# facebook/transform360

Hardware: NVIDIA H100
Metric: Mpixels/s 8K equirect->cubemap bicubic (input-plane pixels consumed per second) (higher is better)
Workload: dtype u8

## Files before the change

### include/transform360_b200.h

```cpp
#ifndef TRANSFORM360_B200_EXT_H
#define TRANSFORM360_B200_EXT_H

#include "Transform360/VideoFrameTransformHandler.h"

#ifdef __cplusplus
extern "C" {
#endif

typedef struct T360HostPlan T360HostPlan;

T360HostPlan* T360B200_hostPlanCreate(const FrameTransformContext* ctx, int inputWidth, int inputHeight,
                                      int outputWidth, int outputHeight);
void T360B200_hostPlanDestroy(T360HostPlan* plan);
int T360B200_hostPlanInfo(const T360HostPlan* plan, int info[6]);
const float* T360B200_hostPlanMap(const T360HostPlan* plan);
const int32_t* T360B200_hostPlanSamples(const T360HostPlan* plan);
int T360B200_hostPlanGather(T360HostPlan* plan, int info[10], const int32_t** jobs, const int32_t** records,
                            const uint32_t** compact);
int T360B200_hostPlanPoleCaps(T360HostPlan* plan, int info[4], const int32_t** capJobs, const uint32_t** capRecords,
                              const int32_t** launchJobs);
int T360B200_dealLanes(int interpolationAlg, int n, const int32_t* phases, int32_t* laneOf, int32_t* copyOf);
int T360B200_weightImage(int interpolationAlg, const uint8_t** image);
int T360B200_hostPlanBlurLists(T360HostPlan* const* plans, int numPlans, int width, int height, int layout[15],
                               const uint8_t** image);
int T360B200_hostPlanSegment(const T360HostPlan* plan, int i, int rect[4], int numTaps[2], const float** kx,
                             const float** ky);
int T360B200_remapTable(int interpolationAlg, const int16_t** table);

int T360B200_transformFramePlaneAsync(VideoFrameTransform* transform, const uint8_t* deviceInput,
                                      uint8_t* deviceOutput, int inputWidth, int inputHeight, int inputPitch,
                                      int outputWidth, int outputHeight, int outputPitch,
                                      int transformMatPlaneIndex, void* cudaStream);
int T360B200_transformFrameAsync(VideoFrameTransform* transform, int numPlanes, const uint8_t* const* deviceInputs,
                                 uint8_t* const* deviceOutputs, const int* inputWidths, const int* inputHeights,
                                 const int* inputPitches, const int* outputWidths, const int* outputHeights,
                                 const int* outputPitches, void* cudaStream);
int T360B200_lowPassPlaneAsync(VideoFrameTransform* transform, const uint8_t* deviceInput, uint8_t* deviceOutput,
                               int width, int height, int inputPitch, int outputPitch,
                               int transformMatPlaneIndex, void* cudaStream);
int T360B200_reconfigure(VideoFrameTransform* transform, const FrameTransformContext* ctx);
typedef struct T360View {
  float yaw, pitch, hfov, vfov;
} T360View;
// ... 33 lines not shown
```

### transform360_b200/build.py

```python
from __future__ import annotations

import os
import shutil
import subprocess
import sys
from pathlib import Path

PKG = Path(__file__).resolve().parent
ROOT = PKG.parent
CSRC = PKG / "csrc"
LIB_DIR = PKG / "lib"
LIB = LIB_DIR / "libTransform360.so"
SOURCES = ["geometry.cpp", "lowpass_plan.cpp", "lowpass_jobs.cpp", "sampling.cpp", "gather_plan.cpp", "kernels.cu", "gather_frame.cu", "view_gather.cu", "video_frame_transform.cpp"]
ARCH = ["-gencode", "arch=compute_90a,code=sm_90a"]


def nvcc_path() -> str:
    p = shutil.which("nvcc") or "/usr/local/cuda/bin/nvcc"
    if not Path(p).exists():
        raise FileNotFoundError("nvcc not found (needed to build libTransform360.so)")
    return p


def needs_build() -> bool:
    if not LIB.exists():
        return True
    t = LIB.stat().st_mtime
    deps = list(CSRC.glob("*")) + list((ROOT / "include").rglob("*.h")) + [Path(__file__)]
    return any(d.stat().st_mtime > t for d in deps)


def build(force: bool = False, verbose: bool = False, defines: tuple = (), out: Path | None = None) -> Path:
    out = out or LIB
    if not force and not defines and not needs_build():
        return LIB
    LIB_DIR.mkdir(exist_ok=True)
# ... 65 lines not shown
```

### transform360_b200/csrc/gather_frame.cu

```cuda
#include "gather_common.cuh"

#include <cuda.h>

#include <algorithm>
#include <cstring>
#include <utility>

namespace t360 {

namespace {

template <class F, int... I>
__device__ __forceinline__ void staticForImpl(F&& f, std::integer_sequence<int, I...>) {
  (f(std::integral_constant<int, I>{}), ...);
}
template <int N, class F>
__device__ __forceinline__ void staticFor(F&& f) {
  staticForImpl(f, std::make_integer_sequence<int, N>{});
}

template <int IMM>
__device__ __forceinline__ uint32_t ldsWordImm(uint32_t addr) {
  uint32_t v;
  asm volatile("ld.shared.u32 %0, [%1+%2];" : "=r"(v) : "r"(addr), "n"(IMM));
// ... 102 lines not shown
  staticFor<8>([&](auto V) {
    constexpr int v = decltype(V)::value;
    const uint4 wt = ldsVecImm<0>(wAddr + (first ^ (uint32_t)(v * kDiagonalStep)));
    const uint32_t b0 = p2 ? B[v ^ 4].b[0] : B[v].b[0], b1 = p2 ? B[v ^ 4].b[1] : B[v].b[1];
    acc = dp2aLo(wt.x, b0, acc); acc = dp2aHi(wt.y, b0, acc);
    acc = dp2aLo(wt.z, b1, acc); acc = dp2aHi(wt.w, b1, acc);
  });
  return acc;
}
template <int K, int VS>
__device__ __forceinline__ int foldPixel(const RowBytes<K> (&W)[K], uint32_t wAddr, uint32_t field) {
  if constexpr (K == 8) return foldRowsRotated<VS>(W, wAddr, field);
  else return foldRows<K, VS>(W, wAddr + slotOffset<K>(field));
}
__device__ __forceinline__ int biasedToByte(int acc) { return min(max(acc >> 15, 0), 255); }


__device__ __forceinline__ uint32_t packBytes(int hi, int lo) {
  uint32_t r;
  asm("cvt.pack.sat.u8.s32.b32 %0, %1, %2, %3;" : "=r"(r) : "r"(hi), "r"(lo), "r"(0));
  return r;
}

template <int K, int PITCH, int VS, int ROWS, bool ZERO>
__device__ __forceinline__ void computeShareJob(uint8_t* dst, int dstPitch, uint32_t stageAddr, const uint4 (&rec)[ROWS / 8],
                                                uint32_t header, uint32_t wAddr) {
  static_assert(PITCH % 4 == 0 && (K == 4 || K == 8) && ROWS % 8 == 0, "");
  uint32_t base = stageAddr + (header & 0x7ffcu);
  const int sh = (int)(header << 3);
  RowBytes<K> W[K];
  staticFor<K>([&](auto R) { W[decltype(R)::value] = loadRow<K, decltype(R)::value * PITCH>(base, sh); });
  int accPrev = 0;
  staticFor<ROWS>([&](auto J) {
    constexpr int j = decltype(J)::value;
    const uint4& block = rec[j >> 3];
    const uint32_t word = ((j >> 1) & 3) == 0 ? block.x : (((j >> 1) & 3) == 1 ? block.y : (((j >> 1) & 3) == 2 ? block.z : block.w));
    const uint32_t r = (j & 1) ? word >> 16 : word;
    if constexpr (j > 0 && !ZERO) {
      const bool two = (r & 1u) != 0;
      const RowBytes<K> below = loadRow<K, (j - 1 + K) * PITCH>(base, sh);
      RowBytes<K> below2 = below;
      if (two) below2 = loadRow<K, (j + K) * PITCH>(base, sh);
#pragma unroll
      for (int q = 0; q + 2 < K; ++q)
#pragma unroll
        for (int i = 0; i < (K == 8 ? 2 : 1); ++i) W[q].b[i] = two ? W[q + 2].b[i] : W[q + 1].b[i];
#pragma unroll
      for (int i = 0; i < (K == 8 ? 2 : 1); ++i) W[K - 2].b[i] = two ? below.b[i] : W[K - 1].b[i];
      W[K - 1] = below2;
      if (two) base += PITCH;
    }
    if constexpr (j > 0 && ZERO) {
      const uint32_t d = r & 3u;
      RowBytes<K> below = W[K - 1], below2 = W[K - 1];
      if (d != 0) below = loadRow<K, K * PITCH>(base, sh);
      if (d == 2) below2 = loadRow<K, (K + 1) * PITCH>(base, sh);
#pragma unroll
      for (int q = 0; q + 2 < K; ++q)
#pragma unroll
        for (int i = 0; i < (K == 8 ? 2 : 1); ++i) W[q].b[i] = d == 0 ? W[q].b[i] : (d == 1 ? W[q + 1].b[i] : W[q + 2].b[i]);
#pragma unroll
      for (int i = 0; i < (K == 8 ? 2 : 1); ++i) {
        W[K - 2].b[i] = d == 0 ? W[K - 2].b[i] : (d == 1 ? W[K - 1].b[i] : below.b[i]);
        W[K - 1].b[i] = d == 0 ? W[K - 1].b[i] : (d == 1 ? below.b[i] : below2.b[i]);
      }
      base += d * PITCH;
    }
    const int acc = foldPixel<K, VS>(W, wAddr, r & kSlotFieldMask) >> 15;
    if constexpr (j & 1) {
      const uint32_t pair = packBytes(acc, accPrev);
      dst[(size_t)(j - 1) * dstPitch] = (uint8_t)pair;
      dst[(size_t)j * dstPitch] = (uint8_t)(pair >> 8);
    } else {
      accPrev = acc;
    }
  });
}

template <int K, int PITCH, int VS>
__device__ __forceinline__ void computeTileJob(const PlaneView& pv, uint32_t stageAddr, int outX, int outY, const uint4& rec,
                                               uint32_t wAddr, int warp) {
  static_assert(PITCH % 4 == 0, "");
  const int y0 = outY + warp * kTilePatchH;
  const int dstPitch = pv.dstPitch, dstW = pv.dstW, dstH = pv.dstH;
  uint8_t* const dstRow = pv.dst + (size_t)y0 * dstPitch + outX;
  const uint32_t words[4] = {rec.x, rec.y, rec.z, rec.w};
  staticFor<kRowsPerPatchStep>([&](auto J) {
    constexpr int j = decltype(J)::value;
    const uint32_t w = words[j];
    const int col = kTilePatchW * j + ((int)(w >> 16) & (kTilePatchW - 1)), row = (int)(w >> 19) & (kTilePatchH - 1);
    if (!(w & kRecordSkip) && outX + col < dstW && y0 + row < dstH) {
// ... 138 lines not shown
      }
      int4 h;
      h.x = __shfl_sync(0xffffffffu, batch.x, pos); h.y = __shfl_sync(0xffffffffu, batch.y, pos);
      h.z = __shfl_sync(0xffffffffu, batch.z, pos); h.w = __shfl_sync(0xffffffffu, batch.w, pos);
      ++pos;
      const int kind = (h.y >> kJobKindShift) & kJobKindMask;
      mbarWait(empty + st, phase ^ 1);
      const bool twoStages = kind == kJobClass1 || kind == kJobSeam;
      if (twoStages) {
        if (st == S - 1) {
          if (lane == 0) postEmptyJob(kJobNop);
          advance();
          mbarWait(empty + st, phase ^ 1);
        }
        mbarWait(empty + st + 1, phase ^ 1);
      }
      if (lane == 0) {
        unsigned char* rec = groupBase + S * kStage + st * kRec;
        *reinterpret_cast<int4*>(rec) = h;
        if (kind == kJobExit) {
          mbarArrive(full + st);
        } else {
          const int pl = h.y >> kJobPlaneShift;
          const uint32_t recBytes = (uint32_t)jobRecordBytes(K, kind, h.x);
          if (kind == kJobBorder) {
            mbarExpectTx(full + st, recBytes);
          } else {
            const int cls = boxClassOf(kind), variant = jobBoxVariant(h.z), boxX = jobBoxX(h.z), boxY = jobBoxY(h.z);
            const uint32_t boxBytes = (uint32_t)(stageBoxW(K, cls) * boxVariantRows(K, cls, variant));
            mbarExpectTx(full + st, (kind == kJobSeam ? 2 : 1) * boxBytes + recBytes);
            tmaLoadBox(groupBase + st * kStage, &maps.map[pl][cls][variant], boxX, boxY, full + st);
            if (kind == kJobSeam)
              tmaLoadBox(groupBase + (st + 1) * kStage, &maps.map[pl][0][variant], boxX - planes[pl].srcW, boxY, full + st);
          }
          bulkCopyToShared(rec + 128, planes[pl].records + (unsigned)h.w, recBytes, full + st);
        }
      }
      advance();
      if (twoStages) {
        if (lane == 0) postEmptyJob(kJobNop);
        advance();
      }
      __syncwarp();
      if (kind == kJobExit) break;
    }
    if (lane == 0 && atomicAdd(jobs.claimCounter + 1, 1) == (int)(gridDim.x * GROUPS) - 1) {
      jobs.claimCounter[0] = 0;
// ... 3 lines not shown
    return;
  }

  const int group = warpId / kGroupWarps, warp = warpId % kGroupWarps;
  unsigned char* groupBase = smem + L::kWeights + group * L::kGroupBytes;
  const uint32_t boxAddr = smemAddr(groupBase), recAddr = smemAddr(groupBase + S * kStage);
  uint64_t* full = barBase + group * 2 * S;
  uint64_t* empty = full + S;
  const uint32_t wAddr = smemAddr(wsmem);
  mbarWait(weightBar, 0);
  asm volatile("griddepcontrol.wait;" ::: "memory");
  auto now = []() { unsigned long long t; asm volatile("mov.u64 %0, %globaltimer;" : "=l"(t)); return t; };
  unsigned long long* trace = jobs.trace && warp == 0 && lane == 0 ? jobs.trace + (size_t)(blockIdx.x * GROUPS + group) * kTraceJobsPerGroup * 4 : nullptr;
  uint32_t traced = 0;
  for (uint32_t st = 0, phase = 0;;) {
    unsigned long long* const row = trace && traced < kTraceJobsPerGroup ? trace + traced * 4 : nullptr;
    if (row) row[0] = now();
    mbarWait(full + st, phase);
    if (row) row[1] = now();
    const uint32_t rec = recAddr + st * kRec;
    const uint4 h = ldsVec(rec);
    const int kind = ((int)h.y >> kJobKindShift) & kJobKindMask;
    if (kind == kJobExit) break;
    const int outX = (int)h.x & ~kJobQuadMask, outY = (int)h.y & kJobRowMask;
    const PlaneView& pv = planes[(int)h.y >> kJobPlaneShift];
    if (kind == kJobShare || kind == kJobShareStay) {
      if constexpr (K >= 4) {
        const uint32_t mine = rec + 128 + warp * shareWarpRecordBytes(K);
        uint4 r[shareRows(K) / 8];
#pragma unroll
        for (int b = 0; b < shareRows(K) / 8; ++b) r[b] = ldsVec(mine + b * 512 + lane * 16);
        const uint32_t header = ldsWord(mine + shareRows(K) / 8 * 512 + lane * 4);
        uint8_t* dst = pv.dst + (size_t)(outY + (warp >> 1) * shareRows(K)) * pv.dstPitch + (outX + (warp & 1) * 32 + (int)(header >> kRecordColumnShift));
        if (kind == kJobShare) computeShareJob<K, stageBoxW(K, 2), VS, shareRows(K), false>(dst, pv.dstPitch, boxAddr + st * kStage, r, header, wAddr);
        else computeShareJob<K, stageBoxW(K, 2), VS, shareRows(K), true>(dst, pv.dstPitch, boxAddr + st * kStage, r, header, wAddr);
      }
    } else if (kind == kJobClass0) {
      uint4 r;
      const int quad = ((int)h.x & kJobQuadMask) - 1;
      if (quad < 0) {
        r = ldsVec(rec + 128 + warp * 512 + lane * 16);
      } else {
        r = make_uint4(kRecordSkip, kRecordSkip, kRecordSkip, kRecordSkip);
        if ((warp >> 2) == (quad >> 1)) {
          const uint2 v = ldsVec2Imm<0>(rec + 128 + (warp & 3) * 256 + lane * 8);
          if (quad & 1) { r.z = v.x; r.w = v.y; } else { r.x = v.x; r.y = v.y; }
        }
      }
      computeTileJob<K, stageBoxW(K, 0), VS>(pv, boxAddr + st * kStage, outX, outY, r, wAddr, warp);
    } else if (kind == kJobClass1) {
      computeTileJob<K, stageBoxW(K, 1), VS>(pv, boxAddr + st * kStage, outX, outY, ldsVec(rec + 128 + warp * 512 + lane * 16), wAddr, warp);
    } else if (kind == kJobSeam) {
      {
        uint4* a = reinterpret_cast<uint4*>(groupBase + st * kStage);
        const uint4* b = reinterpret_cast<const uint4*>(groupBase + (st + 1) * kStage);
        for (int i = warp * 32 + lane; i < (int)(kBox0 / 16); i += kGroupThreads) {
          uint4 x = a[i];
          const uint4 y = b[i];
// ... 83 lines not shown
```

### transform360_b200/csrc/kernels.cuh

```cuda
#pragma once

#include <cuda_runtime.h>

#include <cstdint>

#include "flat_view.h"
#include "oriented_view.h"

namespace t360 {

struct GatherParams {
  const uint8_t* src;
  int srcW, srcH, srcPitch;
  uint8_t* dst;
  int dstW, dstH, dstPitch;
  const int2* samples;
  int tilesPerRow;
  const int16_t* weights;
  int kernelSize;
  int transparent;
};

struct GatherJob {
  int outX, outY;
// ... 63 lines not shown
}
__host__ __device__ constexpr int weightBankGroups(int k) { return k == 2 ? 16 : 8; }
__host__ __device__ constexpr int weightLanesPerPass(int k) { return k == 2 ? 16 : 8; }

__host__ __device__ constexpr int shareWarpRecordBytes(int k) { return shareRows(k) / 8 * 32 * 16 + 32 * 4; }
__host__ __device__ constexpr int shareJobRecordBytes(int k) { return kGroupWarps * shareWarpRecordBytes(k); }
constexpr int kTileJobRecordBytes = kGroupWarps * 32 * 16;
constexpr int kQuadJobRecordBytes = kGroupWarps / 2 * 32 * 8;
__host__ __device__ constexpr int tileJobRecordBytes(int outXField) { return (outXField & kJobQuadMask) ? kQuadJobRecordBytes : kTileJobRecordBytes; }
__host__ __device__ constexpr int stageRecordBytes(int k) {
  return 128 + (shareJobRecordBytes(k) > kTileJobRecordBytes ? shareJobRecordBytes(k) : kTileJobRecordBytes);
}
constexpr int kCapStepBytes = 32 * 8, kBorderPixelBytes = 16;
__host__ __device__ constexpr int capJobMaxSteps(int k) { return (stageRecordBytes(k) - 128) / kCapStepBytes; }
__host__ __device__ constexpr int borderJobMaxPixels(int k) { return (stageRecordBytes(k) - 128) / kBorderPixelBytes; }
__host__ __device__ constexpr int jobRecordBytes(int k, int kind, int outXField) {
  return kind == kJobShare || kind == kJobShareStay ? shareJobRecordBytes(k)
         : kind == kJobCap                          ? outXField * kCapStepBytes
         : kind == kJobBorder                       ? outXField * kBorderPixelBytes
                                                    : tileJobRecordBytes(outXField);
}
constexpr int kRecordColumnShift = 27;

constexpr int kMaxFramePlanes = 3;
struct PlaneView {
  const uint8_t* src;
  uint8_t* dst;
  const uint4* records;
  int srcW, srcH, srcPitch;
  int dstW, dstH, dstPitch;
};
struct FrameGatherParams {
  PlaneView plane[kMaxFramePlanes];
  const uint4* weightImage;
  int kernelSize, numPlanes;
};

__host__ __device__ constexpr int gatherThreads(int k) { return k == 8 ? 512 : 256; }
__host__ __device__ constexpr int gatherTileH(int k) { return gatherThreads(k) / 32 * 4; }

struct StagedParams {
  const GatherJob* tiles;
  int numTiles;
  int* claimCounter;
  unsigned long long* trace;
};
// ... 120 lines not shown
```

### transform360_b200/csrc/video_frame_transform.cpp

```cpp
#include <cuda.h>
#include <cuda_runtime.h>

#include <algorithm>
#include <climits>
#include <cmath>
#include <cstdio>
#include <cstdlib>
#include <cstring>
#include <map>
#include <memory>
#include <mutex>
#include <new>
#include <shared_mutex>
#include <stdexcept>
#include <string>
#include <thread>
#include <vector>

#include "host_plan.h"
#include "gather_plan.h"
#include "kernels.cuh"
#include "lowpass_jobs.h"
#include "transform360_b200.h"

#define T360_API extern "C" __attribute__((visibility("default")))

namespace {

using t360::BlurJob;
using t360::GatherJob;
using t360::HostPlan;
using t360::StripJob;

struct CudaFail {
  cudaError_t err;
  const char* what;
};

#define CU(call)                                       \
  do {                                                 \
    cudaError_t e__ = (call);                          \
    if (e__ != cudaSuccess) throw CudaFail{e__, #call}; \
// ... 1066 lines not shown
      const std::vector<uint8_t> image = t360::buildWeightImage(k, host);
      weightImages_[k].reserve(image.size());
      CU(cudaMemcpy(weightImages_[k].ptr, image.data(), image.size(), cudaMemcpyHostToDevice));
    }
    return buf.ptr;
  }

  DevicePlan upload(HostIndexPlan& p, const FrameTransformContext& ctx) {
    const HostPlan& h = p.host;
    DevicePlan d;
    d.inW = h.inW; d.inH = h.inH; d.outW = h.outW; d.outH = h.outH; d.mapW = h.mapW; d.mapH = h.mapH;
    d.kernelSize = h.kernelSize;
    d.transparent = h.transparentBorder;
    d.stereoFormat = ctx.input_stereo_format;
    if (d.kernelSize > 0) {
      deviceWeights(ctx.interpolation_alg);
      t360::GatherPlan& g = p.gather;
      d.tilesPerRow = g.tilesPerRow;
      d.samples.reserve(g.records.size());
      CU(cudaMemcpy(d.samples.ptr, g.records.data(), g.records.size() * sizeof(int2), cudaMemcpyHostToDevice));
      d.numStaged = g.totalStaged();
      d.numBorder = g.numBorder;
      d.numJobs = static_cast<int>(g.launchJobs.size());
      if (!g.launchJobs.empty()) {
        d.gatherJobs.reserve(g.launchJobs.size());
        CU(cudaMemcpy(d.gatherJobs.ptr, g.launchJobs.data(), g.launchJobs.size() * sizeof(GatherJob), cudaMemcpyHostToDevice));
      }
      if (!g.compact.empty() || !g.capRecords.empty()) {
        d.records.reserve(g.compact.size() + g.capRecords.size());
        if (!g.compact.empty())
          CU(cudaMemcpy(d.records.ptr, g.compact.data(), g.compact.size() * sizeof(uint32_t), cudaMemcpyHostToDevice));
        if (!g.capRecords.empty())
          CU(cudaMemcpy(d.records.ptr + g.compact.size(), g.capRecords.data(), g.capRecords.size() * sizeof(uint32_t), cudaMemcpyHostToDevice));
      }
      d.hostJobs = std::move(g.launchJobs);
      d.jobNeedRows = std::move(g.launchNeedRows);
      d.jobRects = std::move(g.launchRects);
    }
    d.lowPass = ctx.enable_low_pass_filter != 0;
    if (d.lowPass) {
      d.segments = h.segments;
      d.planTaps = h.taps;
      buildBlurSet(d.segments, d.planTaps, h.inW, h.inH, d.stereoFormat, d.blur);
    }
    d.resizeNeeded = h.resize.needed;
    if (d.resizeNeeded) resizeFor(d, d.outW, d.outH);
    if (d.kernelSize > 0 && t360::orientedLayouts(ctx)) {
      const std::vector<float> t = t360::buildSphereTables(t360::sphereGeometry(ctx, h.mapW, h.mapH, h.inW, h.inH, h.kernelSize));
      if (!t.empty()) {
        d.sphereTables.reserve(t.size());
        CU(cudaMemcpy(d.sphereTables.ptr, t.data(), t.size() * sizeof(float), cudaMemcpyHostToDevice));
      }
    }
    return d;
  }

  const DevicePlan::Resize& resizeFor(const DevicePlan& plan, int outW, int outH) {
    std::lock_guard<std::mutex> lock(lazyMu_);
// ... 431 lines not shown

T360_API int VideoFrameTransform_generateMapForPlane(VideoFrameTransform* transform, int inputWidth, int inputHeight,
                                                     int outputWidth, int outputHeight, int transformMatPlaneIndex) {
  if (!transform) return 0;
  return transform->generateMapForPlane(inputWidth, inputHeight, outputWidth, outputHeight, transformMatPlaneIndex);
}

T360_API int VideoFrameTransform_transformFramePlane(VideoFrameTransform* transform, uint8_t* inputData,
                                                     uint8_t* outputData, int inputWidth, int inputHeight,
                                                     int inputWidthWithPadding, int outputWidth, int outputHeight,
                                                     int outputWidthWithPadding, int transformMatPlaneIndex,
                                                     int imagePlaneIndex) {
  if (!transform) return 0;
  return transform->transformFramePlane(inputData, outputData, inputWidth, inputHeight, inputWidthWithPadding,
                                        outputWidth, outputHeight, outputWidthWithPadding, transformMatPlaneIndex,
                                        imagePlaneIndex);
}

struct T360HostPlan {
  HostPlan plan;
  t360::GatherPlan gather;
  bool gatherBuilt = false;
  std::vector<uint8_t> blurImage;
};

T360_API T360HostPlan* T360B200_hostPlanCreate(const FrameTransformContext* ctx, int inW, int inH, int outW, int outH) {
  if (!ctx) return nullptr;
  std::unique_ptr<T360HostPlan> p(new (std::nothrow) T360HostPlan);
  if (!p) return nullptr;
  try {
    if (!t360::buildHostPlan(*ctx, inW, inH, outW, outH, p->plan)) return nullptr;
  } catch (const std::exception& ex) {
    std::printf("Could not build the host plan. Error: %s\n", ex.what());
    return nullptr;
  }
  return p.release();
}
T360_API void T360B200_hostPlanDestroy(T360HostPlan* plan) { delete plan; }
T360_API int T360B200_hostPlanInfo(const T360HostPlan* plan, int info[6]) {
  if (!plan || !info) return 0;
  info[0] = plan->plan.mapW; info[1] = plan->plan.mapH;
  info[2] = static_cast<int>(plan->plan.segments.size());
  info[3] = static_cast<int>(plan->plan.taps.size());
  info[4] = plan->plan.kernelSize;
  info[5] = 0;
  return 1;
// ... 13 lines not shown
  } catch (const std::exception& ex) {
    std::printf("Could not build the gather plan. Error: %s\n", ex.what());
    return 0;
  }
  const t360::GatherPlan& g = plan->gather;
  info[0] = g.tilesPerRow; info[1] = g.tileRows; info[2] = g.tileH; info[3] = static_cast<int>(g.jobs.size());
  info[4] = g.numStaged[0]; info[5] = g.numStaged[1]; info[6] = g.numSeam; info[7] = g.numGeneral;
  info[8] = g.numShare; info[9] = static_cast<int>(g.compact.size());
  if (jobs) *jobs = g.jobs.empty() ? nullptr : reinterpret_cast<const int32_t*>(g.jobs.data());
  if (records) *records = reinterpret_cast<const int32_t*>(g.records.data());
  if (compact) *compact = g.compact.empty() ? nullptr : g.compact.data();
  return 1;
}
T360_API int T360B200_hostPlanPoleCaps(T360HostPlan* plan, int info[4], const int32_t** capJobs, const uint32_t** capRecords,
                                       const int32_t** launchJobs) {
  int gatherInfo[10];
  if (!plan || !info || !T360B200_hostPlanGather(plan, gatherInfo, nullptr, nullptr, nullptr)) return 0;
  const t360::GatherPlan& g = plan->gather;
  info[0] = g.numCap; info[1] = g.numBorder; info[2] = static_cast<int>(g.capRecords.size());
  info[3] = static_cast<int>(g.launchJobs.size());
  if (capJobs) *capJobs = g.capJobs.empty() ? nullptr : reinterpret_cast<const int32_t*>(g.capJobs.data());
  if (capRecords) *capRecords = g.capRecords.empty() ? nullptr : g.capRecords.data();
  if (launchJobs) *launchJobs = g.launchJobs.empty() ? nullptr : reinterpret_cast<const int32_t*>(g.launchJobs.data());
  return 1;
}
T360_API int T360B200_hostPlanBlurLists(T360HostPlan* const* plans, int numPlans, int width, int height, int layout[15],
                                        const uint8_t** image) {
  if (!plans || numPlans < 1 || numPlans > t360::kMaxFramePlanes || !layout || !image) return 0;
  for (int p = 0; p < numPlans; ++p)
    if (!plans[p]) return 0;
  try {
    t360::BlurLists lists[t360::kMaxFramePlanes];
    const t360::BlurLists* planes[t360::kMaxFramePlanes];
    bool clear = false;
    for (int p = 0; p < numPlans; ++p) {
      const HostPlan& h = plans[p]->plan;
      bool c = false;
      t360::buildBlurLists(h.segments, h.taps, width > 0 ? width : h.inW, height > 0 ? height : h.inH, h.ctx.input_stereo_format, lists[p], &c);
      clear = clear || c;
      planes[p] = &lists[p];
    }
    std::vector<uint8_t>& img = plans[0]->blurImage;
    img.clear();
    const t360::BlurLayout l = t360::packBlurLists(numPlans > 1 ? t360::mergeBlurLists(planes, numPlans) : lists[0], img, img);
    const long long v[15] = {l.numStrips[0], l.numStrips[1], l.numStrips[2], l.numTiles, l.numDirect, l.numTaps, l.tileSmem, clear,
                             static_cast<long long>(l.stripAt[0]), static_cast<long long>(l.stripAt[1]), static_cast<long long>(l.stripAt[2]),
// ... 164 lines not shown
```

### transform360_b200/handler.py

```python
from __future__ import annotations

import ctypes as C
import os
from pathlib import Path

import numpy as np

PKG = Path(__file__).resolve().parent
LIB_PATH = PKG / "lib" / "libTransform360.so"

LAYOUT_CUBEMAP_32, LAYOUT_CUBEMAP_23_OFFCENTER, LAYOUT_FLAT_FIXED, LAYOUT_EQUIRECT = 0, 1, 2, 3
LAYOUT_BARREL, LAYOUT_BARREL_SPLIT, LAYOUT_EAC_32, LAYOUT_N = 4, 5, 6, 7
STEREO_FORMAT_TB, STEREO_FORMAT_LR, STEREO_FORMAT_MONO, STEREO_FORMAT_GUESS, STEREO_FORMAT_N = 0, 1, 2, 3, 4
NEAREST, LINEAR, CUBIC, LANCZOS4 = 0, 1, 2, 4


class FrameTransformContext(C.Structure):
    _fields_ = [
        ("input_layout", C.c_int), ("output_layout", C.c_int),
        ("input_stereo_format", C.c_int), ("output_stereo_format", C.c_int),
        ("vflip", C.c_int), ("input_expand_coef", C.c_float), ("expand_coef", C.c_float),
        ("interpolation_alg", C.c_int), ("width_scale_factor", C.c_float),
        ("height_scale_factor", C.c_float), ("fixed_yaw", C.c_float), ("fixed_pitch", C.c_float),
        ("fixed_roll", C.c_float), ("fixed_hfov", C.c_float), ("fixed_vfov", C.c_float),
# ... 63 lines not shown
    L.VideoFrameTransform_delete.argtypes = [vp]
    L.VideoFrameTransform_generateMapForPlane.restype = ci
    L.VideoFrameTransform_generateMapForPlane.argtypes = [vp] + [ci] * 5
    L.VideoFrameTransform_transformFramePlane.restype = ci
    L.VideoFrameTransform_transformFramePlane.argtypes = [vp, vp, vp] + [ci] * 8
    L.T360B200_hostPlanCreate.restype = vp
    L.T360B200_hostPlanCreate.argtypes = [C.POINTER(FrameTransformContext)] + [ci] * 4
    L.T360B200_hostPlanDestroy.restype = None
    L.T360B200_hostPlanDestroy.argtypes = [vp]
    L.T360B200_hostPlanInfo.restype = ci
    L.T360B200_hostPlanInfo.argtypes = [vp, C.POINTER(ci)]
    L.T360B200_hostPlanMap.restype = vp
    L.T360B200_hostPlanMap.argtypes = [vp]
    L.T360B200_hostPlanSamples.restype = vp
    L.T360B200_hostPlanSamples.argtypes = [vp]
    L.T360B200_hostPlanSegment.restype = ci
    L.T360B200_hostPlanSegment.argtypes = [vp, ci, C.POINTER(ci), C.POINTER(ci), C.POINTER(vp), C.POINTER(vp)]
    L.T360B200_hostPlanGather.restype = ci
    L.T360B200_hostPlanGather.argtypes = [vp, C.POINTER(ci), C.POINTER(vp), C.POINTER(vp), C.POINTER(vp)]
    L.T360B200_hostPlanPoleCaps.restype = ci
    L.T360B200_hostPlanBlurLists.restype = ci
    L.T360B200_hostPlanBlurLists.argtypes = [vp, ci, ci, ci, C.POINTER(ci), C.POINTER(vp)]
    L.T360B200_hostPlanPoleCaps.argtypes = [vp, C.POINTER(ci), C.POINTER(vp), C.POINTER(vp), C.POINTER(vp)]
    L.T360B200_weightImage.restype = ci
    L.T360B200_weightImage.argtypes = [ci, C.POINTER(vp)]
    L.T360B200_remapTable.restype = ci
    L.T360B200_remapTable.argtypes = [ci, C.POINTER(vp)]
    L.T360B200_transformFramePlaneAsync.restype = ci
    L.T360B200_transformFramePlaneAsync.argtypes = [vp, vp, vp] + [ci] * 7 + [vp]
    L.T360B200_transformFrameAsync.restype = ci
    L.T360B200_transformFrameAsync.argtypes = [vp, ci, vp, vp] + [vp] * 6 + [vp]
    L.T360B200_lowPassPlaneAsync.restype = ci
    L.T360B200_lowPassPlaneAsync.argtypes = [vp, vp, vp] + [ci] * 5 + [vp]
    L.T360B200_reconfigure.restype = ci
    L.T360B200_reconfigure.argtypes = [vp, C.POINTER(FrameTransformContext)]
    L.T360B200_transformFrameViewAsync.restype = ci
    L.T360B200_transformFrameViewAsync.argtypes = [vp, C.POINTER(T360View), ci, vp, vp] + [vp] * 6 + [vp]
    L.T360B200_viewSamples.restype = ci
    L.T360B200_viewSamples.argtypes = [C.POINTER(FrameTransformContext), C.POINTER(T360View)] + [ci] * 4 + [vp]
    L.T360B200_transformFrameOrientedAsync.restype = ci
    L.T360B200_transformFrameOrientedAsync.argtypes = [vp, C.POINTER(T360Orientation), ci, vp, vp] + [vp] * 6 + [vp]
    L.T360B200_orientedSamples.restype = ci
    L.T360B200_orientedSamples.argtypes = [C.POINTER(FrameTransformContext), C.POINTER(T360Orientation)] + [ci] * 4 + [vp]
    L.T360B200_setPinHostPlanes.restype = None
    L.T360B200_setPinHostPlanes.argtypes = [vp, ci]
    L.T360B200_debugTrace.restype = None
    L.T360B200_debugTrace.argtypes = [vp, ci]
    L.T360B200_debugTraceRead.restype = C.c_ulonglong
    L.T360B200_debugTraceRead.argtypes = [vp, vp, C.c_ulonglong]
    L.T360B200_synchronize.restype = ci
    L.T360B200_synchronize.argtypes = [vp]
    L.T360B200_stream.restype = vp
    L.T360B200_stream.argtypes = [vp]
    L.T360B200_kernelLaunchCount.restype = C.c_ulonglong
    L.T360B200_planDeviceBytes.restype = C.c_ulonglong
    L.T360B200_planDeviceBytes.argtypes = [vp, ci]
    L.T360B200_planTileCounts.restype = ci
    L.T360B200_planTileCounts.argtypes = [vp, ci, C.POINTER(ci)]
    L.T360B200_deviceCount.restype = ci
    L.T360B200_version.restype = C.c_char_p
    if path is None:
        _lib = L
    return L


EXPORTED_SYMBOLS = [
    "VideoFrameTransform_new", "VideoFrameTransform_delete", "VideoFrameTransform_generateMapForPlane",
    "VideoFrameTransform_transformFramePlane", "T360B200_hostPlanCreate", "T360B200_hostPlanDestroy",
    "T360B200_hostPlanInfo", "T360B200_hostPlanMap", "T360B200_hostPlanSamples", "T360B200_hostPlanSegment",
    "T360B200_hostPlanGather", "T360B200_hostPlanPoleCaps", "T360B200_hostPlanBlurLists", "T360B200_weightImage", "T360B200_dealLanes",
    "T360B200_remapTable", "T360B200_transformFramePlaneAsync", "T360B200_transformFrameAsync",
    "T360B200_lowPassPlaneAsync", "T360B200_reconfigure", "T360B200_transformFrameViewAsync", "T360B200_viewSamples",
    "T360B200_transformFrameOrientedAsync", "T360B200_orientedSamples",
    "T360B200_setPinHostPlanes", "T360B200_debugTrace", "T360B200_debugTraceRead", "T360B200_synchronize", "T360B200_stream", "T360B200_kernelLaunchCount", "T360B200_planDeviceBytes",
    "T360B200_planTileCounts", "T360B200_deviceCount", "T360B200_version",
]


class VideoFrameTransform:

    def __init__(self, ctx: FrameTransformContext):
        self._lib = load()
        self.ctx = ctx
        self._h = self._lib.VideoFrameTransform_new(C.byref(ctx))
        if not self._h:
            raise MemoryError("VideoFrameTransform_new returned NULL")

    def close(self):
        if getattr(self, "_h", None):
            self._lib.VideoFrameTransform_delete(self._h)
            self._h = None

    __del__ = close
# ... 150 lines not shown
        if not self._lib.T360B200_hostPlanGather(self._h, info, C.byref(jobs), C.byref(recs), C.byref(comp)):
            raise ValueError("T360B200_hostPlanGather failed")
        tpr, trows, th, nj = info[0], info[1], info[2], info[3]
        n = tpr * trows * th * 32 * 2
        records = np.frombuffer((C.c_int32 * n).from_address(recs.value), np.int32).reshape(tpr * trows, th, 32, 2).copy()
        j = compact = None
        if nj and jobs.value:
            j = np.frombuffer((C.c_int32 * (nj * 4)).from_address(jobs.value), np.int32).reshape(nj, 4).copy()
        if info[9] and comp.value:
            compact = np.frombuffer((C.c_uint32 * info[9]).from_address(comp.value), np.uint32).copy()
        return dict(tiles_per_row=tpr, tile_rows=trows, tile_h=th, jobs=j, records=records, compact=compact,
                    counts=dict(class0=info[4], class1=info[5], seam=info[6], general=info[7], share=info[8]))

    def pole_caps(self):
        info = (C.c_int * 4)()
        jobs, recs, launch = C.c_void_p(), C.c_void_p(), C.c_void_p()
        if not self._lib.T360B200_hostPlanPoleCaps(self._h, info, C.byref(jobs), C.byref(recs), C.byref(launch)):
            raise ValueError("T360B200_hostPlanPoleCaps failed")
        n, m = info[0] + info[1], info[3]
        as_jobs = lambda p, k: np.frombuffer((C.c_int32 * (k * 4)).from_address(p.value), np.int32).reshape(k, 4).copy() if k and p.value else np.zeros((0, 4), np.int32)
        records = np.frombuffer((C.c_uint32 * info[2]).from_address(recs.value), np.uint32).copy() if info[2] and recs.value else np.zeros(0, np.uint32)
        return dict(counts=dict(cap=info[0], border=info[1]), jobs=as_jobs(jobs, n), records=records, launch=as_jobs(launch, m))

    def blur_lists(self, *others, width=0, height=0):
        plans = (C.c_void_p * (1 + len(others)))(self._h, *[o._h for o in others])
        lay, img = (C.c_int * 15)(), C.c_void_p()
        if not self._lib.T360B200_hostPlanBlurLists(plans, len(plans), width, height, lay, C.byref(img)):
            raise ValueError("T360B200_hostPlanBlurLists failed (message on stdout)")
        image = C.string_at(img.value, lay[14]) if lay[14] else b""
        arr = lambda at, n, cols, dt: np.frombuffer(image, dt, n * cols, at).reshape(n, cols).copy()
        return dict(image=image, strips=[arr(lay[8 + c], lay[c], 9, np.int32) for c in range(3)], tiles=arr(lay[11], lay[3], 8, np.int32),
                    direct=arr(lay[12], lay[4], 8, np.int32), taps=np.frombuffer(image, np.float32, lay[5], lay[13]).copy(),
                    offsets=list(lay[8:14]), tile_smem=lay[6], needs_clear=bool(lay[7]))

    def segments(self):
        out = []
        rect, nk = (C.c_int * 4)(), (C.c_int * 2)()
        kx, ky = C.c_void_p(), C.c_void_p()
        for i in range(self.num_segments):
            assert self._lib.T360B200_hostPlanSegment(self._h, i, rect, nk, C.byref(kx), C.byref(ky))
            a = np.frombuffer((C.c_float * nk[0]).from_address(kx.value), np.float32).copy()
            b = np.frombuffer((C.c_float * nk[1]).from_address(ky.value), np.float32).copy()
            out.append((rect[0], rect[1], rect[2], rect[3], a, b))
        return out


# ... 56 lines not shown
```

Measured before the change: 730,900.

## Pack bicubic share-job records into compact per-lane bytes for device streaming

Adds a host-side pass that re-encodes share-job records for the bicubic (K=4) path. For each warp whose rows share one column phase, the per-row 16-bit slot fields become 8-bit step/fracY bytes, with the column phase folded into the header. The kernel decodes these packed records and keeps the old layout only for 'wide' warps, which are flagged by a bitmask in the job's outX. This cuts the record bytes fetched per job into shared memory, at the cost of extra decode ALU work and a 16-bit limit on output columns. It also adds a traffic-measurement script.

```diff
diff --git a/include/transform360_b200.h b/include/transform360_b200.h
--- a/include/transform360_b200.h
+++ b/include/transform360_b200.h
@@ -19,6 +19,7 @@
                             const uint32_t** compact);
 int T360B200_hostPlanPoleCaps(T360HostPlan* plan, int info[4], const int32_t** capJobs, const uint32_t** capRecords,
                               const int32_t** launchJobs);
+int T360B200_hostPlanDeviceRecords(T360HostPlan* plan, int info[2], const int32_t** launchJobs, const uint32_t** words);
 int T360B200_dealLanes(int interpolationAlg, int n, const int32_t* phases, int32_t* laneOf, int32_t* copyOf);
 int T360B200_weightImage(int interpolationAlg, const uint8_t** image);
 int T360B200_hostPlanBlurLists(T360HostPlan* const* plans, int numPlans, int width, int height, int layout[15],
diff --git a/profiles/record_traffic.py b/profiles/record_traffic.py
--- /dev/null
+++ b/profiles/record_traffic.py
@@ -0,0 +1,83 @@
+from __future__ import annotations
+
+import argparse
+import json
+import statistics
+import subprocess
+import sys
+from pathlib import Path
+
+ROOT = Path(__file__).resolve().parents[1]
+sys.path.insert(0, str(ROOT))
+
+
+def gpu_info():
+    q = subprocess.run(["nvidia-smi", "-i", "0", "--query-gpu=name,power.limit,clocks.max.sm", "--format=csv,noheader,nounits"],
+                       capture_output=True, text=True).stdout.strip().split(", ")
+    return {"gpu": q[0], "power_limit_w": float(q[1]), "sm_max_mhz": float(q[2])} if len(q) == 3 else {"gpu": None, "power_limit_w": None}
+
+
+def main():
+    ap = argparse.ArgumentParser()
+    ap.add_argument("--config", default="cfg2", choices=["cfg2", "cfg3", "cfg4"])
+    ap.add_argument("--frames", type=int, default=500, help="frames per timed window")
+    ap.add_argument("--rounds", type=int, default=5, help="alternated windows of each condition")
+    ap.add_argument("--label", default="", help="free text stored with the line (e.g. which build)")
+    ap.add_argument("--out", help="append the JSON line to this file")
+    args = ap.parse_args()
+    import torch
+    import transform360_b200 as t360
+    from bench import CONFIGS
+    from transform360_b200 import synth
+    from transform360_b200.stream import FrameTransformer, StreamSpec
+
+    if not torch.cuda.is_available():
+        sys.exit("needs a CUDA device")
+    info = gpu_info()
+    cfg = CONFIGS[args.config]
+    spec = StreamSpec(cfg["inp"][0], cfg["inp"][1], cfg["out"][0], cfg["out"][1])
+    ft = FrameTransformer(t360.make_context(**dict(cfg["ov"], enable_low_pass_filter=0)), spec)
+    pitch = lambda w: (w + 255) // 256 * 256
+    ring = max(4, -(-200_000_000 // spec.input_pixels_per_frame()))
+    d_in = [[synth.noise_plane_torch(*spec.plane_dims(p)[:2], plane=p, frame=f, device="cuda", pitch=pitch(spec.plane_dims(p)[0]))
+             for p in range(3)] for f in range(ring)]
+    d_out = [[torch.zeros((spec.plane_dims(p)[3], pitch(spec.plane_dims(p)[2])), dtype=torch.uint8, device="cuda") for p in range(3)]
+             for _ in range(2)]
+    args_of = lambda planes: [(t.data_ptr(), t.stride(0)) for t in planes]
+    calls = [[ft.frame_call(args_of(d_in[i]), args_of(d_out[o])) for o in range(2)] for i in range(ring)]
+    st = torch.cuda.Stream()
+
+    def window(repeat):
+        for i in range(10):
+            assert calls[0 if repeat else i % ring][i % 2](st.cuda_stream)
+        a, b = torch.cuda.Event(enable_timing=True), torch.cuda.Event(enable_timing=True)
+        a.record(st)
+        for i in range(args.frames):
+            assert calls[0 if repeat else i % ring][i % 2](st.cuda_stream)
+        b.record(st)
+        b.synchronize()
+        return a.elapsed_time(b) / args.frames
+
+    torch.cuda.synchronize()
+    times = {"ring": [], "repeat": []}
+    for _ in range(args.rounds):
+        times["ring"].append(window(False))
+        times["repeat"].append(window(True))
+    summary = {k: {"ms": [round(x, 5) for x in v], "median_ms": round(statistics.median(v), 5), "min_ms": round(min(v), 5),
+                   "max_ms": round(max(v), 5)} for k, v in times.items()}
+    separated = summary["repeat"]["max_ms"] < summary["ring"]["min_ms"]
+    line = dict(info, label=args.label, config=args.config, frames=args.frames, rounds=args.rounds, ring_frames=ring,
+                input_bytes_per_frame=spec.input_pixels_per_frame(), output_bytes_per_frame=spec.output_pixels_per_frame(),
+                plan_device_bytes=[ft.vft.plan_device_bytes(i) for i in (0, 1)], conditions=summary,
+                repeat_faster_outside_spread=separated,
+                repeat_saving=round(1 - summary["repeat"]["median_ms"] / summary["ring"]["median_ms"], 4))
+    ft.close()
+    out = json.dumps(line)
+    print(out)
+    if args.out:
+        with open(args.out, "a") as f:
+            f.write(out + "\n")
+
+
+if __name__ == "__main__":
+    main()
diff --git a/transform360_b200/build.py b/transform360_b200/build.py
--- a/transform360_b200/build.py
+++ b/transform360_b200/build.py
@@ -11,7 +11,7 @@
 CSRC = PKG / "csrc"
 LIB_DIR = PKG / "lib"
 LIB = LIB_DIR / "libTransform360.so"
-SOURCES = ["geometry.cpp", "lowpass_plan.cpp", "lowpass_jobs.cpp", "sampling.cpp", "gather_plan.cpp", "kernels.cu", "gather_frame.cu", "view_gather.cu", "video_frame_transform.cpp"]
+SOURCES = ["geometry.cpp", "lowpass_plan.cpp", "lowpass_jobs.cpp", "sampling.cpp", "gather_plan.cpp", "device_records.cpp", "kernels.cu", "gather_frame.cu", "view_gather.cu", "video_frame_transform.cpp"]
 ARCH = ["-gencode", "arch=compute_90a,code=sm_90a"]
 
 
diff --git a/transform360_b200/csrc/device_records.cpp b/transform360_b200/csrc/device_records.cpp
--- /dev/null
+++ b/transform360_b200/csrc/device_records.cpp
@@ -0,0 +1,71 @@
+#include "device_records.h"
+
+#include <climits>
+#include <stdexcept>
+
+namespace t360 {
+namespace {
+
+constexpr uint32_t kFracYBits = 0x3e00;
+
+uint32_t shareRecord(const uint32_t* warp, int lane, int j) { return (warp[lane * 4 + (j >> 1)] >> (16 * (j & 1))) & 0xffffu; }
+
+uint32_t columnPhase(int k, uint32_t columnField) {
+  const int copy = static_cast<int>(columnField >> 14) & 1, inCopy = static_cast<int>(columnField >> 4) & 31;
+  const int slot = copy ? ((inCopy & ~7) | ((inCopy - copy) & 7)) : inCopy;
+  const int fracX = ((slot & 15) << 1) | ((slot >> 4) & 1);
+  if (static_cast<uint32_t>(weightSlotField(k, fracX, copy)) != columnField) throw std::logic_error("device records: not a slot field");
+  return static_cast<uint32_t>(fracX | (copy << 5));
+}
+
+unsigned packShareJob(int k, const uint32_t* job, std::vector<uint32_t>& out) {
+  unsigned wide = 0;
+  for (int w = 0; w < kGroupWarps; ++w) {
+    const uint32_t* warp = job + static_cast<size_t>(w) * (shareWarpRecordBytes(k) / 4);
+    for (int lane = 0; lane < 32 && !(wide >> w & 1u); ++lane)
+      for (int j = 1; j < shareRows(k); ++j)
+        if ((shareRecord(warp, lane, j) ^ shareRecord(warp, lane, 0)) & kSlotFieldMask & ~kFracYBits) wide |= 1u << w;
+    if (wide >> w & 1u) {
+      out.insert(out.end(), warp, warp + shareWarpRecordBytes(k) / 4);
+      continue;
+    }
+    const uint32_t* headers = warp + shareRows(k) / 8 * 32 * 4;
+    for (int lane = 0; lane < 32; ++lane) {
+      uint32_t bytes[2] = {0, 0};
+      for (int j = 0; j < shareRows(k); ++j) {
+        const uint32_t r = shareRecord(warp, lane, j);
+        if (r & ~(kSlotFieldMask | 3u)) throw std::logic_error("device records: share step out of range");
+        bytes[j >> 2] |= (((r & kFracYBits) >> 9) << 3 | (r & 3u)) << (8 * (j & 3));
+      }
+      out.push_back(bytes[0]);
+      out.push_back(bytes[1]);
+    }
+    for (int lane = 0; lane < 32; ++lane) {
+      const uint32_t phase = columnPhase(k, shareRecord(warp, lane, 0) & kSlotFieldMask & ~kFracYBits);
+      out.push_back(headers[lane] | (phase & 31u) << kShareFracXShift | (phase >> 5) << kShareCopyShift);
+    }
+  }
+  return wide;
+}
+
+}
+
+void buildDeviceRecords(const GatherPlan& g, int k, DeviceRecords& out) {
+  out = DeviceRecords{};
+  out.launchJobs = g.launchJobs;
+  for (GatherJob& job : out.launchJobs) {
+    const int kind = (job.outY >> kJobKindShift) & kJobKindMask;
+    const size_t at = static_cast<size_t>(job.recordOffset) * 4;
+    const uint32_t* src = at < g.compact.size() ? &g.compact[at] : &g.capRecords[at - g.compact.size()];
+    job.recordOffset = static_cast<int>(out.words.size() / 4);
+    if (sharePacked(k) && (kind == kJobShare || kind == kJobShareStay)) {
+      if (job.outX >> kJobShareWideShift) throw std::invalid_argument("device records: share jobs hold 16-bit output columns");
+      job.outX |= static_cast<int>(packShareJob(k, src, out.words)) << kJobShareWideShift;
+    } else {
+      out.words.insert(out.words.end(), src, src + jobRecordBytes(k, kind, job.outX) / 4);
+    }
+    if (out.words.size() / 4 > static_cast<size_t>(INT32_MAX)) throw std::invalid_argument("device records: offsets overflow");
+  }
+}
+
+}
diff --git a/transform360_b200/csrc/device_records.h b/transform360_b200/csrc/device_records.h
--- /dev/null
+++ b/transform360_b200/csrc/device_records.h
@@ -0,0 +1,17 @@
+#pragma once
+
+#include <cstdint>
+#include <vector>
+
+#include "gather_plan.h"
+
+namespace t360 {
+
+struct DeviceRecords {
+  std::vector<GatherJob> launchJobs;
+  std::vector<uint32_t> words;
+};
+
+void buildDeviceRecords(const GatherPlan& g, int k, DeviceRecords& out);
+
+}
diff --git a/transform360_b200/csrc/gather_frame.cu b/transform360_b200/csrc/gather_frame.cu
--- a/transform360_b200/csrc/gather_frame.cu
+++ b/transform360_b200/csrc/gather_frame.cu
@@ -148,10 +148,36 @@
   return r;
 }
 
-template <int K, int PITCH, int VS, int ROWS, bool ZERO>
-__device__ __forceinline__ void computeShareJob(uint8_t* dst, int dstPitch, uint32_t stageAddr, const uint4 (&rec)[ROWS / 8],
+struct CompactShareRecords {
+  uint4 r;
+  template <int j>
+  __device__ __forceinline__ uint32_t rec() const {
+    const uint32_t word = (j >> 1) == 0 ? r.x : ((j >> 1) == 1 ? r.y : ((j >> 1) == 2 ? r.z : r.w));
+    return (j & 1) ? word >> 16 : word;
+  }
+  template <int j>
+  __device__ __forceinline__ uint32_t field() const { return rec<j>() & kSlotFieldMask; }
+  template <int j>
+  __device__ __forceinline__ uint32_t step() const { return rec<j>(); }
+};
+struct PackedShareRecords {
+  uint2 b;
+  uint32_t columnField;
+  template <int j>
+  __device__ __forceinline__ uint32_t field() const {
+    constexpr int s = 8 * (j & 3) + 3 - 9;
+    const uint32_t word = j < 4 ? b.x : b.y;
+    return ((s >= 0 ? word >> s : word << -s) & 0x3e00u) | columnField;
+  }
+  template <int j>
+  __device__ __forceinline__ uint32_t step() const { return (j < 4 ? b.x : b.y) >> (8 * (j & 3)); }
+};
+
+template <int K, int PITCH, int VS, bool ZERO, class Records>
+__device__ __forceinline__ void computeShareJob(uint8_t* dst, int dstPitch, uint32_t stageAddr, const Records& rec,
                                                 uint32_t header, uint32_t wAddr) {
-  static_assert(PITCH % 4 == 0 && (K == 4 || K == 8) && ROWS % 8 == 0, "");
+  constexpr int ROWS = 8;
+  static_assert(PITCH % 4 == 0 && (K == 4 || K == 8) && shareRows(K) == ROWS, "");
   uint32_t base = stageAddr + (header & 0x7ffcu);
   const int sh = (int)(header << 3);
   RowBytes<K> W[K];
@@ -159,9 +185,7 @@
   int accPrev = 0;
   staticFor<ROWS>([&](auto J) {
     constexpr int j = decltype(J)::value;
-    const uint4& block = rec[j >> 3];
-    const uint32_t word = ((j >> 1) & 3) == 0 ? block.x : (((j >> 1) & 3) == 1 ? block.y : (((j >> 1) & 3) == 2 ? block.z : block.w));
-    const uint32_t r = (j & 1) ? word >> 16 : word;
+    const uint32_t r = rec.template step<j>();
     if constexpr (j > 0 && !ZERO) {
       const bool two = (r & 1u) != 0;
       const RowBytes<K> below = loadRow<K, (j - 1 + K) * PITCH>(base, sh);
@@ -192,7 +216,7 @@
       }
       base += d * PITCH;
     }
-    const int acc = foldPixel<K, VS>(W, wAddr, r & kSlotFieldMask) >> 15;
+    const int acc = foldPixel<K, VS>(W, wAddr, rec.template field<j>()) >> 15;
     if constexpr (j & 1) {
       const uint32_t pair = packBytes(acc, accPrev);
       dst[(size_t)(j - 1) * dstPitch] = (uint8_t)pair;
@@ -377,7 +401,7 @@
           mbarArrive(full + st);
         } else {
           const int pl = h.y >> kJobPlaneShift;
-          const uint32_t recBytes = (uint32_t)jobRecordBytes(K, kind, h.x);
+          const uint32_t recBytes = (uint32_t)deviceJobRecordBytes(K, kind, h.x);
           if (kind == kJobBorder) {
             mbarExpectTx(full + st, recBytes);
           } else {
@@ -427,18 +451,31 @@
     const uint4 h = ldsVec(rec);
     const int kind = ((int)h.y >> kJobKindShift) & kJobKindMask;
     if (kind == kJobExit) break;
-    const int outX = (int)h.x & ~kJobQuadMask, outY = (int)h.y & kJobRowMask;
+    const int outX = (int)h.x & kJobOutXMask, outY = (int)h.y & kJobRowMask;
     const PlaneView& pv = planes[(int)h.y >> kJobPlaneShift];
     if (kind == kJobShare || kind == kJobShareStay) {
       if constexpr (K >= 4) {
-        const uint32_t mine = rec + 128 + warp * shareWarpRecordBytes(K);
-        uint4 r[shareRows(K) / 8];
-#pragma unroll
-        for (int b = 0; b < shareRows(K) / 8; ++b) r[b] = ldsVec(mine + b * 512 + lane * 16);
-        const uint32_t header = ldsWord(mine + shareRows(K) / 8 * 512 + lane * 4);
-        uint8_t* dst = pv.dst + (size_t)(outY + (warp >> 1) * shareRows(K)) * pv.dstPitch + (outX + (warp & 1) * 32 + (int)(header >> kRecordColumnShift));
-        if (kind == kJobShare) computeShareJob<K, stageBoxW(K, 2), VS, shareRows(K), false>(dst, pv.dstPitch, boxAddr + st * kStage, r, header, wAddr);
-        else computeShareJob<K, stageBoxW(K, 2), VS, shareRows(K), true>(dst, pv.dstPitch, boxAddr + st * kStage, r, header, wAddr);
+        constexpr int PITCH = stageBoxW(K, 2);
+        const uint32_t wide = h.x >> kJobShareWideShift;
+        const uint32_t mine = sharePacked(K) ? rec + 128 + warp * kPackedShareWarpBytes + __popc(wide & ((1u << warp) - 1u)) * shareWideExtraBytes(K)
+                                             : rec + 128 + warp * shareWarpRecordBytes(K);
+        const uint32_t stageAddr = boxAddr + st * kStage;
+        if (sharePacked(K) && !((wide >> warp) & 1u)) {
+          PackedShareRecords r;
+          r.b = ldsVec2Imm<0>(mine + lane * 8);
+          const uint32_t header = ldsWord(mine + 256 + lane * 4);
+          r.columnField = (uint32_t)weightSlotField(K, (header >> kShareFracXShift) & 31u, (header >> kShareCopyShift) & 1u);
+          uint8_t* dst = pv.dst + (size_t)(outY + (warp >> 1) * shareRows(K)) * pv.dstPitch + (outX + (warp & 1) * 32 + (int)(header >> kRecordColumnShift));
+          if (kind == kJobShare) computeShareJob<K, PITCH, VS, false>(dst, pv.dstPitch, stageAddr, r, header, wAddr);
+          else computeShareJob<K, PITCH, VS, true>(dst, pv.dstPitch, stageAddr, r, header, wAddr);
+        } else {
+          CompactShareRecords r;
+          r.r = ldsVec(mine + lane * 16);
+          const uint32_t header = ldsWord(mine + 512 + lane * 4);
+          uint8_t* dst = pv.dst + (size_t)(outY + (warp >> 1) * shareRows(K)) * pv.dstPitch + (outX + (warp & 1) * 32 + (int)(header >> kRecordColumnShift));
+          if (kind == kJobShare) computeShareJob<K, PITCH, VS, false>(dst, pv.dstPitch, stageAddr, r, header, wAddr);
+          else computeShareJob<K, PITCH, VS, true>(dst, pv.dstPitch, stageAddr, r, header, wAddr);
+        }
       }
     } else if (kind == kJobClass0) {
       uint4 r;
diff --git a/transform360_b200/csrc/kernels.cuh b/transform360_b200/csrc/kernels.cuh
--- a/transform360_b200/csrc/kernels.cuh
+++ b/transform360_b200/csrc/kernels.cuh
@@ -109,6 +109,22 @@
 }
 constexpr int kRecordColumnShift = 27;
 
+__host__ __device__ constexpr bool sharePacked(int k) { return k == 4; }
+constexpr int kShareFracXShift = 16, kShareCopyShift = 21, kJobShareWideShift = 16;
+constexpr int kJobOutXMask = 0xffff & ~kJobQuadMask;
+constexpr int kPackedShareWarpBytes = 32 * 8 + 32 * 4;
+static_assert(shareRows(4) == 8 && shareRows(8) == 8, "packed share records hold 8 rows per warp");
+__host__ __device__ constexpr int shareWideExtraBytes(int k) { return shareWarpRecordBytes(k) - kPackedShareWarpBytes; }
+__host__ __device__ constexpr int packedShareJobRecordBytes(int k, unsigned wideMask) {
+  int n = 0;
+  for (; wideMask; wideMask &= wideMask - 1) ++n;
+  return kGroupWarps * kPackedShareWarpBytes + n * shareWideExtraBytes(k);
+}
+__host__ __device__ constexpr int deviceJobRecordBytes(int k, int kind, int outXField) {
+  return sharePacked(k) && (kind == kJobShare || kind == kJobShareStay) ? packedShareJobRecordBytes(k, (unsigned)outXField >> kJobShareWideShift)
+                                                                        : jobRecordBytes(k, kind, outXField);
+}
+
 constexpr int kMaxFramePlanes = 3;
 struct PlaneView {
   const uint8_t* src;
diff --git a/transform360_b200/csrc/video_frame_transform.cpp b/transform360_b200/csrc/video_frame_transform.cpp
--- a/transform360_b200/csrc/video_frame_transform.cpp
+++ b/transform360_b200/csrc/video_frame_transform.cpp
@@ -18,6 +18,7 @@
 #include <vector>
 
 #include "host_plan.h"
+#include "device_records.h"
 #include "gather_plan.h"
 #include "kernels.cuh"
 #include "lowpass_jobs.h"
@@ -1130,18 +1131,17 @@
       d.numStaged = g.totalStaged();
       d.numBorder = g.numBorder;
       d.numJobs = static_cast<int>(g.launchJobs.size());
-      if (!g.launchJobs.empty()) {
-        d.gatherJobs.reserve(g.launchJobs.size());
-        CU(cudaMemcpy(d.gatherJobs.ptr, g.launchJobs.data(), g.launchJobs.size() * sizeof(GatherJob), cudaMemcpyHostToDevice));
-      }
-      if (!g.compact.empty() || !g.capRecords.empty()) {
-        d.records.reserve(g.compact.size() + g.capRecords.size());
-        if (!g.compact.empty())
-          CU(cudaMemcpy(d.records.ptr, g.compact.data(), g.compact.size() * sizeof(uint32_t), cudaMemcpyHostToDevice));
-        if (!g.capRecords.empty())
-          CU(cudaMemcpy(d.records.ptr + g.compact.size(), g.capRecords.data(), g.capRecords.size() * sizeof(uint32_t), cudaMemcpyHostToDevice));
-      }
-      d.hostJobs = std::move(g.launchJobs);
+      t360::DeviceRecords dr;
+      t360::buildDeviceRecords(g, d.kernelSize, dr);
+      if (!dr.launchJobs.empty()) {
+        d.gatherJobs.reserve(dr.launchJobs.size());
+        CU(cudaMemcpy(d.gatherJobs.ptr, dr.launchJobs.data(), dr.launchJobs.size() * sizeof(GatherJob), cudaMemcpyHostToDevice));
+      }
+      if (!dr.words.empty()) {
+        d.records.reserve(dr.words.size());
+        CU(cudaMemcpy(d.records.ptr, dr.words.data(), dr.words.size() * sizeof(uint32_t), cudaMemcpyHostToDevice));
+      }
+      d.hostJobs = std::move(dr.launchJobs);
       d.jobNeedRows = std::move(g.launchNeedRows);
       d.jobRects = std::move(g.launchRects);
     }
@@ -1619,6 +1619,8 @@
   t360::GatherPlan gather;
   bool gatherBuilt = false;
   std::vector<uint8_t> blurImage;
+  t360::DeviceRecords deviceRecords;
+  bool deviceRecordsBuilt = false;
 };
 
 T360_API T360HostPlan* T360B200_hostPlanCreate(const FrameTransformContext* ctx, int inW, int inH, int outW, int outH) {
@@ -1678,6 +1680,25 @@
   if (capJobs) *capJobs = g.capJobs.empty() ? nullptr : reinterpret_cast<const int32_t*>(g.capJobs.data());
   if (capRecords) *capRecords = g.capRecords.empty() ? nullptr : g.capRecords.data();
   if (launchJobs) *launchJobs = g.launchJobs.empty() ? nullptr : reinterpret_cast<const int32_t*>(g.launchJobs.data());
+  return 1;
+}
+T360_API int T360B200_hostPlanDeviceRecords(T360HostPlan* plan, int info[2], const int32_t** launchJobs, const uint32_t** words) {
+  int gatherInfo[10];
+  if (!plan || !info || !T360B200_hostPlanGather(plan, gatherInfo, nullptr, nullptr, nullptr)) return 0;
+  try {
+    if (!plan->deviceRecordsBuilt) {
+      t360::buildDeviceRecords(plan->gather, plan->plan.kernelSize, plan->deviceRecords);
+      plan->deviceRecordsBuilt = true;
+    }
+  } catch (const std::exception& ex) {
+    std::printf("Could not build the device records. Error: %s\n", ex.what());
+    return 0;
+  }
+  const t360::DeviceRecords& d = plan->deviceRecords;
+  info[0] = static_cast<int>(d.launchJobs.size());
+  info[1] = static_cast<int>(d.words.size());
+  if (launchJobs) *launchJobs = d.launchJobs.empty() ? nullptr : reinterpret_cast<const int32_t*>(d.launchJobs.data());
+  if (words) *words = d.words.empty() ? nullptr : d.words.data();
   return 1;
 }
 T360_API int T360B200_hostPlanBlurLists(T360HostPlan* const* plans, int numPlans, int width, int height, int layout[15],
diff --git a/transform360_b200/handler.py b/transform360_b200/handler.py
--- a/transform360_b200/handler.py
+++ b/transform360_b200/handler.py
@@ -109,6 +109,8 @@
     L.T360B200_hostPlanBlurLists.restype = ci
     L.T360B200_hostPlanBlurLists.argtypes = [vp, ci, ci, ci, C.POINTER(ci), C.POINTER(vp)]
     L.T360B200_hostPlanPoleCaps.argtypes = [vp, C.POINTER(ci), C.POINTER(vp), C.POINTER(vp), C.POINTER(vp)]
+    L.T360B200_hostPlanDeviceRecords.restype = ci
+    L.T360B200_hostPlanDeviceRecords.argtypes = [vp, C.POINTER(ci), C.POINTER(vp), C.POINTER(vp)]
     L.T360B200_weightImage.restype = ci
     L.T360B200_weightImage.argtypes = [ci, C.POINTER(vp)]
     L.T360B200_remapTable.restype = ci
@@ -155,7 +157,7 @@
     "VideoFrameTransform_new", "VideoFrameTransform_delete", "VideoFrameTransform_generateMapForPlane",
     "VideoFrameTransform_transformFramePlane", "T360B200_hostPlanCreate", "T360B200_hostPlanDestroy",
     "T360B200_hostPlanInfo", "T360B200_hostPlanMap", "T360B200_hostPlanSamples", "T360B200_hostPlanSegment",
-    "T360B200_hostPlanGather", "T360B200_hostPlanPoleCaps", "T360B200_hostPlanBlurLists", "T360B200_weightImage", "T360B200_dealLanes",
+    "T360B200_hostPlanGather", "T360B200_hostPlanPoleCaps", "T360B200_hostPlanDeviceRecords", "T360B200_hostPlanBlurLists", "T360B200_weightImage", "T360B200_dealLanes",
     "T360B200_remapTable", "T360B200_transformFramePlaneAsync", "T360B200_transformFrameAsync",
     "T360B200_lowPassPlaneAsync", "T360B200_reconfigure", "T360B200_transformFrameViewAsync", "T360B200_viewSamples",
     "T360B200_transformFrameOrientedAsync", "T360B200_orientedSamples",
@@ -352,6 +354,16 @@
         records = np.frombuffer((C.c_uint32 * info[2]).from_address(recs.value), np.uint32).copy() if info[2] and recs.value else np.zeros(0, np.uint32)
         return dict(counts=dict(cap=info[0], border=info[1]), jobs=as_jobs(jobs, n), records=records, launch=as_jobs(launch, m))
 
+    def device_records(self):
+        info = (C.c_int * 2)()
+        launch, words = C.c_void_p(), C.c_void_p()
+        if not self._lib.T360B200_hostPlanDeviceRecords(self._h, info, C.byref(launch), C.byref(words)):
+            raise ValueError("T360B200_hostPlanDeviceRecords failed (message on stdout)")
+        m, n = info[0], info[1]
+        jobs = np.frombuffer((C.c_int32 * (m * 4)).from_address(launch.value), np.int32).reshape(m, 4).copy() if m and launch.value else np.zeros((0, 4), np.int32)
+        recs = np.frombuffer((C.c_uint32 * n).from_address(words.value), np.uint32).copy() if n and words.value else np.zeros(0, np.uint32)
+        return dict(launch=jobs, words=recs)
+
     def blur_lists(self, *others, width=0, height=0):
         plans = (C.c_void_p * (1 + len(others)))(self._h, *[o._h for o in others])
         lay, img = (C.c_int * 15)(), C.c_void_p()
```

Result: no change. 732,100, median of 6 (+0.2%).
